# liaoherui/StrainScan

Hardware: AMD Instinct MI355X
Metric: M reads/sec vs 1433-strain E. coli DB (higher is better)
Workload: dtype u64

## Files before the change

### strainscan_amd/csrc/ss_common.h

```cpp
#pragma once
#include <hip/hip_runtime.h>
#include <stdint.h>
#include <stdio.h>
#include <atomic>
#include <functional>
#include <vector>
#include <string.h>

#include "strainscan_hip.h"

namespace ss {

void set_last_error(const char *what, const char *file, int line, hipError_t e);

#define SS_HIP(call)                                               \
    do {                                                           \
        hipError_t _e = (call);                                    \
        if (_e != hipSuccess) {                                    \
            ss::set_last_error(#call, __FILE__, __LINE__, _e);     \
            return (_e == hipErrorOutOfMemory) ? SS_ENOMEM         \
                   : (_e == hipErrorNoDevice)  ? SS_ENODEV         \
                                               : SS_EHIP;          \
        }                                                          \
    } while (0)
// ... 51 lines not shown
    uint32_t n_dir = 0;
    uint32_t n_dir_alloc = 0;
    uint32_t *d_bloom = nullptr;
    uint32_t bloom_bits = 0;
    uint64_t n_buckets = 0;
    uint32_t *d_counts = nullptr;
    int expect_hits = 0;
    uint64_t probe_set = 0;
    int probe_comb = 0;
    double probe_runs_per_tile = 0;
    uint32_t *d_slot_of_row = nullptr;
    uint8_t *d_row_valid = nullptr;
    char *h_stage[2] = {nullptr, nullptr};
    char *d_stage[2] = {nullptr, nullptr};
    uint64_t stage_bytes = 0;
    hipStream_t streams[2] = {nullptr, nullptr};
    hipEvent_t stage_free[2] = {nullptr, nullptr};
    std::atomic<uint64_t> launches{0};
    struct Worker { char *h_buf = nullptr; char *d_buf = nullptr; hipEvent_t done = nullptr; uint64_t cap = 0;
                    char *t_buf = nullptr; uint64_t t_cap = 0; };
    static constexpr int MAX_WORKERS = 64;
    Worker workers[MAX_WORKERS];
    static void free_workers(Worker *w, int n);
    uint64_t device_bytes = 0;
};

#include <chrono>
#include <mutex>

namespace ss { hipError_t big_malloc(void **p, uint64_t bytes, uint64_t *got = nullptr); void big_put(void *p, uint64_t cap); }
struct ss_reads {
    struct Slab {
        char *d = nullptr; uint64_t cap = 0, used = 0; bool binned = false;
        bool packed = false; uint64_t n_pos = 0; uint32_t L = 0, slot = 0;
        uint64_t positions() const { return packed ? n_pos : used; }
    };
    std::vector<Slab> slabs;
    std::mutex mu;
    uint64_t n_records = 0, n_bases = 0, device_bytes = 0, n_blocks = 0;
    bool has_cut_record = false;
    uint64_t first_slab = 0;
    uint64_t serial = next_serial();
    static uint64_t next_serial() { static std::atomic<uint64_t> c{0}; return ++c; }

    static uint64_t padded(uint64_t len) { return (len + 1 + 15) & ~15ull; }
    void adopt(char *d, uint64_t cap, uint64_t len)
    {
        std::lock_guard<std::mutex> g(mu);
        Slab sl;
        sl.d = d; sl.cap = cap; sl.used = padded(len);
        if (!slabs.empty() && slabs.back().used < slabs.back().cap) slabs.insert(slabs.end() - 1, sl);
        else slabs.push_back(sl);
        device_bytes += cap;
        n_blocks++;
    }
    char *reserve(uint64_t len)
    {
        const uint64_t need = padded(len);
        std::lock_guard<std::mutex> g(mu);
        if (slabs.empty() || slabs.back().used + need > slabs.back().cap) {
            Slab sl;
            sl.cap = std::max<uint64_t>(need, slabs.empty() ? std::max<uint64_t>(first_slab, 64ull << 20) : 512ull << 20);
            const auto t0 = std::chrono::steady_clock::now();
            if (ss::big_malloc((void **)&sl.d, sl.cap, &sl.cap) != hipSuccess) return nullptr;
            if (getenv("SS_INGEST_TRACE"))
                fprintf(stderr, "[ingest] slab of %.0f MB: %.4f s\n", sl.cap / 1e6,
                        std::chrono::duration<double>(std::chrono::steady_clock::now() - t0).count());
            slabs.push_back(sl);
        }
        Slab &sl = slabs.back();
        char *p = sl.d + sl.used;
        sl.used += need;
        device_bytes += need;
        n_blocks++;
        return p;
    }
};


namespace ss {
int reads_order_for_locality(ss_reads *R, bool force = false);
int order_flat_dev(const char *src, uint64_t n, ss_reads::Slab *out);
extern std::atomic<long long> g_hook_ascii_slabs;
void reorder_release();
void reorder_counters(uint64_t out[2]);
void reorder_timing(double out[3]);
int build_mini(ss_db *db, const uint64_t *keys, const uint8_t *flags, uint64_t n_rows, int upper_keys);
int build_mini_dev(ss_db *db, const uint64_t *keys, const uint8_t *flags, uint64_t n_rows, int upper_keys);
int mark_solid(ss_db *db);
using BlockSink = std::function<int(const char *h_buf, char *d_buf, uint64_t len, hipStream_t stream)>;
int parse_file_parallel(ss_db::Worker *workers, const char *path, int shard_rank, int shard_world,
                        uint64_t *n_records, uint64_t *n_bases, bool *handled, const BlockSink &sink, bool copy = true);
int parse_text_parallel(ss_db::Worker *workers, const char *text, uint64_t n, const char *path, int shard_rank,
                        int shard_world, uint64_t *n_records, uint64_t *n_bases, bool *handled, const BlockSink &sink,
                        bool copy = true);
struct InflatedText { char *p = nullptr; uint64_t n = 0; };
bool inflate_whole(const char *path, uint64_t budget, char **text, uint64_t *len, int mode, unsigned threads);
uint64_t inflate_budget_bytes();
hipStream_t ingest_stream(unsigned i);
void free_later(char *p);
std::vector<InflatedText> inflate_gz_inputs(const char *const *paths, int n_paths);
bool gz_on_gpu();
int gz_policy();
bool gpu_gunzip(const uint8_t *in, uint64_t in_n, char **text_dev, uint64_t *len, void **lease, int fd);
void gpu_gunzip_done(void *lease);
hipStream_t call_stream_get();
void call_stream_put(hipStream_t s);
struct GzPiece { uint64_t at, len, keep; std::vector<uint8_t> carry; };
bool gz_range_active();
extern std::atomic<long long> g_hook_entry, g_hook_decline, g_hook_skip_chain;
uint64_t gz_range_ticket();
void gz_range_pass(uint64_t ticket);
bool gpu_gunzip_range(const uint8_t *in, uint64_t in_n, char **text_dev, void **lease, int fd, std::vector<GzPiece> *pieces,
                      uint64_t ticket, bool decline = false);
int gz_fastq_pieces_dev(const char *path, uint64_t ticket, const std::function<int(char *, uint64_t, uint64_t, uint64_t)> &flat);
int gz_fastq_to_flat_dev(const char *path, int shard_rank, int shard_world, char **d_flat, uint64_t *flat_len, uint64_t *flat_cap,
                         uint64_t *n_records, char **text, uint64_t *text_len);
int gz_inputs_on_device(const char *const *paths, int n_paths, int shard_rank, int shard_world,
                        const std::function<int(int, char *, uint64_t, uint64_t, uint64_t)> &flat, std::vector<InflatedText> &texts,
                        std::vector<char> &done);
int scan_file_parallel(ss_db *db, const char *path, uint64_t *n_records, uint64_t *n_bases, bool *handled, int shard_rank = 0,
                       int shard_world = 1);
int scan_text_parallel(ss_db *db, const char *text, uint64_t n, uint64_t *n_records, uint64_t *n_bases, bool *handled,
                       int shard_rank = 0, int shard_world = 1);
int launch_scan_mini(ss_db *db, const void *bases_dev, uint64_t n, hipStream_t stream, unsigned blocks,
                     uint64_t n_tiles, bool binned = false, uint64_t set_id = 0, bool packed = false);
int launch_scan_mini_multi(ss_db *const *dbs, int n_dbs, const void *bases_dev, uint64_t n, hipStream_t stream, bool binned,
                           bool packed = false);
enum { MULTI_BLOOM = 0, MULTI_EXPECT = 1, MULTI_PLAIN = 2 };
int multi_kind(const ss_db *db);
void pool_keep_at_least(uint64_t bytes);
namespace l2s {
inline hipStream_t stream() { return hipStreamPerThread; }
hipError_t dmalloc(void **p, size_t n);
inline hipError_t dfree(void *p) { return p ? hipFreeAsync(p, stream()) : hipSuccess; }
inline hipError_t copy(void *d, const void *s_, size_t n, hipMemcpyKind k)
{
    const hipError_t e = hipMemcpyAsync(d, s_, n, k, stream());
    return e != hipSuccess ? e : hipStreamSynchronize(stream());
}
inline hipError_t set(void *d, int v, size_t n) { return hipMemsetAsync(d, v, n, stream()); }
inline hipError_t sync() { return hipStreamSynchronize(stream()); }
}
constexpr uint64_t BIG_KEEP_MIN = 256ull << 20;
void *big_take(uint64_t bytes, uint64_t *cap = nullptr);
void big_put(void *p, uint64_t cap);
void big_release();
hipError_t big_malloc(void **p, uint64_t bytes, uint64_t *got);
bool upload_file_to_device(int fd, uint64_t n, uint8_t *d_dst);
int scan_flat_dev(ss_db *db, const void *bases_dev, uint64_t n, void *stream, bool binned, uint64_t set_id = 0, bool packed = false);
}
```

### strainscan_amd/csrc/ss_ginflate.hip

```cpp
#include "ss_common.h"

#include <fcntl.h>
#include <sys/stat.h>
#include <unistd.h>
#include <zlib.h>

#include <algorithm>
#include <chrono>
#include <atomic>
#include <condition_variable>
#include <mutex>
#include <thread>
#include <vector>
#include <functional>
#include <future>

namespace {

constexpr uint32_t WSIZE = 32768;
constexpr uint16_t UNRES = 0x8000;
#ifndef SS_GZ_RING
#define SS_GZ_RING 2048
#endif
#ifndef SS_GZ_LITBITS
// ... 2338 lines not shown
    static const uint8_t hdr[10] = {0x1f, 0x8b, 8, 0, 0, 0, 0, 0, 0, 0xff};
    memcpy(img.get(), hdr, 10);
    {
        const unsigned T = (unsigned)std::max<uint64_t>(1, std::min<uint64_t>(8, comp_n >> 24));
        std::atomic<bool> ok(true);
        std::vector<std::thread> pool;
        for (unsigned w = 0; w < T; w++)
            pool.emplace_back([&, w] {
                uint64_t a = comp_n * w / T;
                const uint64_t e = comp_n * (w + 1) / T;
                while (a < e) {
                    const ssize_t r = pread(fd, img.get() + 10 + a, (size_t)std::min<uint64_t>(e - a, 1u << 30), (off_t)(off + a));
                    if (r <= 0) { ok = false; return; }
                    a += (uint64_t)r;
                }
            });
        for (auto &th : pool) th.join();
        close(fd);
        if (!ok) { delete L; return SS_EIO; }
    }
    uint8_t *t8 = img.get() + 10 + comp_n;
    for (int q = 0; q < 4; q++) { t8[q] = (uint8_t)(crc >> (8 * q)); t8[4 + q] = (uint8_t)(usize >> (8 * q)); }
    char *d = nullptr;
    uint64_t len = 0;
    if (!ss::gpu_gunzip(img.get(), in_n, &d, &len, &L->gz, -1)) { delete L; return SS_ERANGE; }
    if (len != usize) { ss::gpu_gunzip_done(L->gz); delete L; return SS_EIO; }
    *d_data = d; *n = len; *lease = L;
    return SS_OK;
}
extern "C" int ss_npz_member_done(void *lease)
{
    NpzLease *L = static_cast<NpzLease *>(lease);
    if (!L) return SS_OK;
    if (L->gz) ss::gpu_gunzip_done(L->gz);
    if (L->d_buf) hipFree(L->d_buf);
    delete L;
    return SS_OK;
}

extern "C" int ss_crc32_repeat(uint32_t prefix_crc, int byte, uint64_t n, uint32_t *out)
{
    if (!out || byte < 0 || byte > 255) return SS_EINVAL;
    const unsigned char b = (unsigned char)byte;
    uLong pw = crc32(crc32(0L, Z_NULL, 0), &b, 1);
    uLong acc = prefix_crc;
    uint64_t len = 1;
    for (uint64_t m = n; m; m >>= 1, len <<= 1) {
        if (m & 1) acc = crc32_combine(acc, pw, (z_off_t)len);
        if (m >> 1) pw = crc32_combine(pw, pw, (z_off_t)len);
    }
    *out = (uint32_t)acc;
    return SS_OK;
}

extern "C" int ss_gz_warm_up(int n_files)
{
    std::vector<PinSet *> got;
    for (int i = 0; i < std::min(n_files, 2); i++) {
        PinSet *p = pin_get();
        if (!p) break;
        got.push_back(p);
    }
    const bool ok = (int)got.size() == std::min(n_files, 2);
    for (PinSet *p : got) pin_put(p);
    return ok ? SS_OK : SS_ENOMEM;
}

extern "C" int ss_gz_set_range(int rank, int world, uint64_t slice_bytes, ss_gz_chain_fn chain, void *user)
{
    if (world < 1 || rank < 0 || rank >= world) return SS_EINVAL;
    std::lock_guard<std::mutex> one(ss::g_range_mu);
    ss::g_range.rank = rank; ss::g_range.world = world; ss::g_range.slice_bytes = slice_bytes; ss::g_range.fn = chain; ss::g_range.user = user;
    return SS_OK;
}

extern "C" int ss_test_hook(int which, long long value)
{
    switch (which) {
    case 1: ss::g_hook_entry = value; return SS_OK;
    case 2: ss::g_hook_decline = value; return SS_OK;
    case 3: ss::g_hook_skip_chain = value; return SS_OK;
    case 4: ss::g_hook_generic_k = value; return SS_OK;
    case 5: ss::g_hook_ascii_slabs = value; return SS_OK;
    default: return SS_EINVAL;
    }
}

extern "C" int ss_gz_range_counters(uint64_t *files, uint64_t *pieces)
{
    if (files) *files = ss::g_range_files.load();
    if (pieces) *pieces = ss::g_range_pieces.load();
    return SS_OK;
}
```

### strainscan_amd/csrc/ss_reorder.hip

```cpp
#include "ss_common.h"

#include <mutex>
#include "ss_scan_dev.h"

#include <algorithm>
#include <chrono>
#include <vector>

namespace {

#ifndef SS_ORDER_CH
#define SS_ORDER_CH 64
#endif
constexpr int CH = SS_ORDER_CH;
constexpr int RB = 256 * CH;
constexpr int HALO = 512;
static_assert(22 <= 23, "a table entry has 24 bits for the bin; order_bits stays at or below 22");
constexpr uint32_t NO_NL = 0xFFFFFFFFu;
constexpr int TCAP = 2 * CH;

__device__ __forceinline__ uint32_t nl_mask16(const uint4 v)
{
    const uint32_t w[4] = {v.x, v.y, v.z, v.w};
    uint32_t z[4];
#pragma unroll
    for (int d = 0; d < 4; d++) {
        const uint32_t x = w[d] ^ 0x0A0A0A0Au;
        z[d] = ~(((x & 0x7F7F7F7Fu) + 0x7F7F7F7Fu) | x) & 0x80808080u;
    }
    const uint32_t lo = __builtin_amdgcn_udot4(z[1], 0x80402010u, __builtin_amdgcn_udot4(z[0], 0x08040201u, 0u, false), false);
    const uint32_t hi = __builtin_amdgcn_udot4(z[3], 0x80402010u, __builtin_amdgcn_udot4(z[2], 0x08040201u, 0u, false), false);
    return (lo >> 7) | ((hi >> 7) << 8);
}

__device__ __forceinline__ uint4 load16_nl(const char *__restrict__ b, uint64_t i, uint64_t n)
{
    if (i + 16 <= n) { uint4 v; __builtin_memcpy(&v, b + i, 16); return v; }
    uint32_t w[4] = {0x0A0A0A0Au, 0x0A0A0A0Au, 0x0A0A0A0Au, 0x0A0A0A0Au};
    for (int k = 0; k < 16 && i + k < n; k++) {
        const uint32_t ch = (uint8_t)b[i + k];
        w[k >> 2] = (w[k >> 2] & ~(0xFFu << (8 * (k & 3)))) | (ch << (8 * (k & 3)));
    }
    return make_uint4(w[0], w[1], w[2], w[3]);
}

__device__ __forceinline__ uint32_t record_bin(const char *__restrict__ b, uint64_t s, uint64_t len, int bits)
{
    if (len < 31) return 1u << bits;
    uint4 q[2];
    __builtin_memcpy(q, b + s, 32);
    const uint32_t w[8] = {q[0].x, q[0].y, q[0].z, q[0].w, q[1].x, q[1].y, q[1].z, q[1].w};
    uint64_t km = 0;
    uint32_t bad = 0;
#pragma unroll
    for (int d = 0; d < 8; d++) {
        const uint32_t c = (w[d] >> 1) & 0x03030303u;
        const uint32_t letter = __builtin_amdgcn_perm(0u, 0x47544341u, c);
        uint32_t diff = (w[d] & 0xDFDFDFDFu) ^ letter;
        if (d == 7) diff &= 0x00FFFFFFu;
        bad |= diff;
        km |= (uint64_t)__builtin_amdgcn_udot4(c, 0x40100401u, 0u, false) << (8 * d);
    }
    if (bad) return 1u << bits;
    km &= 0x3FFFFFFFFFFFFFFFull;
    uint32_t best = 0xFFFFFFFFu;
#pragma unroll
    for (int i = 0; i < 31 - ss::MINI_M + 1; i++) {
        const uint32_t x = (uint32_t)(km >> (2 * i));
        best = min(best, (ss::mmkey(x) & ss::KEY_MASK) | (uint32_t)i);
    }
    const uint32_t x = (uint32_t)(km >> (2 * (best & 31u))) & ss::M30;
    return ss::mix30(x) >> (30 - bits);
}

__device__ __forceinline__ uint32_t wave_incl_sum(uint32_t v, int lane)
{
#pragma unroll
    for (int off = 1; off < 64; off <<= 1) {
        const uint32_t o = (uint32_t)__shfl_up((int)v, off, 64);
        if (lane >= off) v += o;
    }
    return v;
}

constexpr uint32_t T_OVERFLOW = 0xFFFFFFFFu;
constexpr int START_BITS = CH == 64 ? 14 : 15, LEN_BITS = 40 - START_BITS;
constexpr uint32_t LEN_LIMIT = 1u << LEN_BITS;
static_assert(RB == 1 << START_BITS, "a table entry holds the start within the tile in START_BITS bits");

struct TileLds {
    uint32_t first[5];
    uint32_t wcnt[4];
    uint32_t more;
    uint64_t src[256], dst[256];
    uint32_t len[256], bin[256], pend[256];
};

#if SS_ORDER_CH == 128
typedef unsigned __int128 mask_t;
__device__ __forceinline__ uint32_t mask_ctz(mask_t m) { const uint64_t lo = (uint64_t)m; return lo ? (uint32_t)__builtin_ctzll(lo) : 64u + (uint32_t)__builtin_ctzll((uint64_t)(m >> 64)); }
#else
typedef uint64_t mask_t;
__device__ __forceinline__ uint32_t mask_ctz(mask_t m) { return (uint32_t)__builtin_ctzll(m); }
#endif
struct TileState { mask_t nl, st; uint32_t later; uint64_t tile0, i0; };

__device__ __forceinline__ void tile_setup(const char *__restrict__ b, uint64_t n, TileLds &L, TileState &S)
{
    const int t = threadIdx.x, lane = t & 63, wave = t >> 6;
    S.tile0 = (uint64_t)blockIdx.x * RB;
    S.i0 = S.tile0 + (uint64_t)t * CH;
    mask_t nl = ~(mask_t)0;
    uint32_t prev = 1u;
    if (S.i0 < n) {
        uint4 v[CH / 16];
#pragma unroll
        for (int k = 0; k < CH / 16; k++) v[k] = load16_nl(b, S.i0 + 16u * k, n);
        prev = S.i0 == 0 ? 1u : (uint32_t)(b[S.i0 - 1] == '\n');
        nl = 0;
#pragma unroll
        for (int k = 0; k < CH / 16; k++) nl |= (mask_t)nl_mask16(v[k]) << (16 * k);
    }
    uint32_t suf = nl ? (uint32_t)t * CH + mask_ctz(nl) : NO_NL;
#pragma unroll
    for (int off = 1; off < 64; off <<= 1) {
        const uint32_t o = (uint32_t)__shfl_down((int)suf, off, 64);
// ... 339 lines not shown
            if (p < total) store_piece(dst, (((uint64_t)hi << 32) | lo) + off[r], v[r], L, slot, off[r]);
        }
    }
}

constexpr uint32_t PK_LDS = 4352;
constexpr int FPK = 4;

__global__ __launch_bounds__(256, 6) void place_fixed_packed_kernel(const char *__restrict__ b, uint64_t n, uint64_t n_rec, uint32_t L,
                                                                    uint32_t P, uint32_t magic_p, uint32_t A, uint32_t G, uint32_t ND,
                                                                    uint32_t magic_nd, unsigned long long *__restrict__ cursor,
                                                                    const uint32_t *__restrict__ bins, uint8_t *__restrict__ dst)
{
    __shared__ uint32_t lds[4][PK_LDS / 4 + 1];
    const int lane = threadIdx.x & 63, wave = threadIdx.x >> 6;
    const uint64_t r0 = ((uint64_t)blockIdx.x * 4u + (uint32_t)wave) * 64u;
    if (r0 >= n_rec) return;
    const uint32_t L1 = L + 1u, nr = (uint32_t)min((uint64_t)64, n_rec - r0), slot = slot_of(L), B = slot / 8u * 3u;
    const uint64_t base = r0 * L1;
    uint32_t *W = lds[wave];
    uint8_t *W8 = reinterpret_cast<uint8_t *>(W);
    unsigned long long d0 = 0;
    if ((uint32_t)lane < nr) d0 = atomicAdd(&cursor[bins[r0 + lane]], (unsigned long long)slot);
    for (uint32_t c0 = 0; c0 < nr; c0 += G) {
        const uint32_t nc = min(G, nr - c0), total = nc * P;
        for (uint32_t p0 = 0; p0 < total; p0 += 64u * FPK) {
            uint4 v[FPK];
#pragma unroll
            for (int r = 0; r < FPK; r++) {
                const uint32_t p = p0 + (uint32_t)lane + 64u * r, rec = min(__umulhi(p, magic_p), nc - 1u), off = (p - rec * P) * 16u;
                v[r] = make_uint4(0x0A0A0A0Au, 0x0A0A0A0Au, 0x0A0A0A0Au, 0x0A0A0A0Au);
                if (p < total && L > off) v[r] = load16_nl(b, base + (uint64_t)(c0 + rec) * L1 + off, n);
            }
#pragma unroll
            for (int r = 0; r < FPK; r++) {
                const uint32_t p = p0 + (uint32_t)lane + 64u * r, rec = min(__umulhi(p, magic_p), nc - 1u), off = (p - rec * P) * 16u;
                if (p >= total) continue;
                uint32_t w[4] = {v[r].x, v[r].y, v[r].z, v[r].w};
                const int keep = (int)min(16u, L > off ? L - off : 0u);
                if (keep < 16) {
#pragma unroll
                    for (int d = 0; d < 4; d++) {
                        const int k = keep - 4 * d;
                        if (k <= 0) w[d] = 0x0A0A0A0Au;
                        else if (k < 4) { const uint32_t m = (1u << (8 * k)) - 1u; w[d] = (w[d] & m) | (0x0A0A0A0Au & ~m); }
                    }
                }
                uint32_t code, inv;
                ss::dev::encode16(w, code, inv);
                uint16_t *q = reinterpret_cast<uint16_t *>(W8 + rec * A + 4u + (off >> 4) * 6u);
                q[0] = (uint16_t)code;
                q[1] = (uint16_t)((inv & 0xFFu) | ((code >> 8) & 0xFF00u));
                q[2] = (uint16_t)((code >> 24) | (inv & 0xFF00u));
            }
        }
        __builtin_amdgcn_fence(__ATOMIC_RELEASE, "wavefront");
        __builtin_amdgcn_wave_barrier();
        __builtin_amdgcn_fence(__ATOMIC_ACQUIRE, "wavefront");
        const uint32_t items = nc * ND;
        for (uint32_t i0 = 0; i0 < items; i0 += 64u) {
            const uint32_t i = i0 + (uint32_t)lane, rec = min(__umulhi(i, magic_nd), nc - 1u), jl = i - rec * ND;
            const uint32_t lo = (uint32_t)__shfl((int)(uint32_t)d0, (int)(c0 + rec), 64), hi = (uint32_t)__shfl((int)(uint32_t)(d0 >> 32), (int)(c0 + rec), 64);
            const uint64_t D = ((((uint64_t)hi << 32) | lo) >> 3) * 3u;
            const int o = (int)(4u * jl) - (int)(D & 3u);
            if (i < items && o < (int)B) {
                const uint32_t x = rec * A + 4u + (uint32_t)o;
                const uint32_t val = __builtin_amdgcn_alignbyte(W[(x >> 2) + 1u], W[x >> 2], x & 3u);
                uint8_t *out = dst + (D & ~3ull) + 4u * jl;
                if (o >= 0 && o + 4 <= (int)B) {
                    *reinterpret_cast<uint32_t *>(__builtin_assume_aligned(out, 4)) = val;
                } else {
#pragma unroll
                    for (int k = 0; k < 4; k++)
                        if (o + k >= 0 && o + k < (int)B) out[k] = (uint8_t)(val >> (8 * k));
                }
            }
        }
        __builtin_amdgcn_fence(__ATOMIC_RELEASE, "wavefront");
        __builtin_amdgcn_wave_barrier();
        __builtin_amdgcn_fence(__ATOMIC_ACQUIRE, "wavefront");
    }
}

constexpr int SCAN_PER = 4096;

__global__ __launch_bounds__(1024) void scan_sums_kernel(const unsigned long long *__restrict__ v, uint32_t n, unsigned long long *__restrict__ sums)
{
    __shared__ unsigned long long s_w[16];
    const int t = threadIdx.x, lane = t & 63, wave = t >> 6;
    const uint32_t i0 = blockIdx.x * SCAN_PER + (uint32_t)t * 4u;
    unsigned long long x = 0;
    for (uint32_t i = i0; i < min(n, i0 + 4u); i++) x += v[i];
#pragma unroll
    for (int off = 32; off > 0; off >>= 1) x += (unsigned long long)__shfl_xor((long long)x, off, 64);
    if (lane == 0) s_w[wave] = x;
    __syncthreads();
    if (t == 0) { unsigned long long r = 0; for (int w = 0; w < 16; w++) r += s_w[w]; sums[blockIdx.x] = r; }
}

__global__ __launch_bounds__(1024) void scan_top_kernel(unsigned long long *__restrict__ sums, uint32_t nb, unsigned long long *__restrict__ total)
{
    __shared__ unsigned long long s_part[1024];
    const int t = threadIdx.x;
    const uint32_t per = (nb + 1023u) / 1024u, a = min(nb, (uint32_t)t * per), e = min(nb, a + per);
    unsigned long long sum = 0;
    for (uint32_t i = a; i < e; i++) sum += sums[i];
    s_part[t] = sum;
    __syncthreads();
    if (t == 0) {
        unsigned long long run = 0;
        for (int i = 0; i < 1024; i++) { const unsigned long long v = s_part[i]; s_part[i] = run; run += v; }
        *total = run;
    }
    __syncthreads();
    unsigned long long run = s_part[t];
    for (uint32_t i = a; i < e; i++) { const unsigned long long v = sums[i]; sums[i] = run; run += v; }
}

__global__ __launch_bounds__(1024) void scan_apply_kernel(unsigned long long *__restrict__ v, uint32_t n, const unsigned long long *__restrict__ sums)
{
    __shared__ unsigned long long s_w[16];
    const int t = threadIdx.x, lane = t & 63, wave = t >> 6;
    const uint32_t i0 = blockIdx.x * SCAN_PER + (uint32_t)t * 4u;
    unsigned long long x[4], mine = 0;
#pragma unroll
    for (int k = 0; k < 4; k++) { x[k] = i0 + k < n ? v[i0 + k] : 0ull; mine += x[k]; }
    unsigned long long incl = mine;
#pragma unroll
    for (int off = 1; off < 64; off <<= 1) {
        const unsigned long long o = (unsigned long long)__shfl_up((long long)incl, off, 64);
        if (lane >= off) incl += o;
    }
    if (lane == 63) s_w[wave] = incl;
    __syncthreads();
    unsigned long long run = sums[blockIdx.x] + incl - mine;
    for (int w = 0; w < wave; w++) run += s_w[w];
#pragma unroll
    for (int k = 0; k < 4; k++) { if (i0 + k < n) v[i0 + k] = run; run += x[k]; }
}

int order_bits(uint64_t n_bytes)
{
    int bits = 12;
    while (bits < 22 && (n_bytes / 152) >> (bits + 2)) bits++;
    return bits;
}

}

namespace ss {

static std::mutex g_scr_mu;
static uint64_t g_order_n[2] = {0, 0};
static double g_order_ms[3] = {0, 0, 0};
static char *g_scr = nullptr;
static uint64_t g_scr_cap = 0;

std::atomic<long long> g_hook_ascii_slabs{0};

int order_flat_dev(const char *src, uint64_t n, ss_reads::Slab *out)
{
    *out = ss_reads::Slab();
    const int bits = order_bits(n);
    const uint32_t n_bins = (1u << bits) + 1u;
    static const bool trace = getenv("SS_INGEST_TRACE") != nullptr;
    const auto t_begin = std::chrono::steady_clock::now();
    auto lap = [&](const char *what) {
        if (!trace) return;
        hipDeviceSynchronize();
        fprintf(stderr, "[reorder] %-22s at %.4f s\n", what, std::chrono::duration<double>(std::chrono::steady_clock::now() - t_begin).count());
    };
    const unsigned nb = (unsigned)((n + RB - 1) / RB), nsb = (n_bins + SCAN_PER - 1) / SCAN_PER;
    const uint64_t o_sums = ((uint64_t)n_bins + 3) * 8, o_cnt = o_sums + (((uint64_t)nsb + 1) * 8), o_tab = (o_cnt + (uint64_t)nb * 4 + 255) & ~255ull;
    uint32_t fix_L = 0;
    uint64_t n_rec = 0;
    static const bool fixed_allowed = [] { const char *e = getenv("SS_ORDER_FIXED"); return !(e && !strcmp(e, "0")); }();
    if (fixed_allowed && n >= 64) {
        char head[FIX_MAX_L + 2];
        const size_t hn = (size_t)std::min<uint64_t>(n, sizeof(head));
        if (hipMemcpy(head, src, hn, hipMemcpyDeviceToHost) != hipSuccess) { ss::set_last_error("hipMemcpy", __FILE__, __LINE__, hipGetLastError()); return SS_EHIP; }
        const void *nl = memchr(head, '\n', hn);
        if (nl) {
            const uint32_t L = (uint32_t)((const char *)nl - head);
            if (L >= FIX_MIN_L && L <= FIX_MAX_L && n / (L + 1) >= 1 && n - (n / (L + 1)) * (L + 1) < 64) { fix_L = L; n_rec = n / (L + 1); }
        }
    }
    const uint64_t scratch = o_tab + std::max<uint64_t>((uint64_t)nb * TCAP * 8, (n_rec * 4 + 255) & ~255ull);
    char *d_scr = nullptr, *d_new = nullptr;
#define SS_R(call) do { if ((call) != hipSuccess) { ss::set_last_error(#call, __FILE__, __LINE__, hipGetLastError()); hipFree(d_scr); hipFree(d_new); return SS_EHIP; } } while (0)
    uint64_t scr_cap = 0;
    {
        std::lock_guard<std::mutex> g(g_scr_mu);
        if (g_scr && g_scr_cap >= scratch) { d_scr = g_scr; scr_cap = g_scr_cap; g_scr = nullptr; g_scr_cap = 0; }
    }
    if (!d_scr) { SS_R(hipMalloc((void **)&d_scr, scratch)); scr_cap = scratch; }
    unsigned long long *d_hist = (unsigned long long *)d_scr, *d_sums = (unsigned long long *)(d_scr + o_sums);
    uint32_t *d_cnt = (uint32_t *)(d_scr + o_cnt);
    unsigned long long *d_tab = (unsigned long long *)(d_scr + o_tab);
    constexpr unsigned pad1 = 0, pad2 = 0;
    unsigned long long tail[3] = {0, 0, 0};
    bool fixed = false, packed = false;
    if (fix_L) {
        const uint32_t L1 = fix_L + 1u, P = (::slot_of(fix_L) + 15u) >> 4;
        const unsigned nbf = (unsigned)((n_rec + 255) / 256);
        SS_R(hipMemsetAsync(d_hist, 0, o_sums, 0));
        hipLaunchKernelGGL(count_fixed_kernel, dim3(nbf), dim3(256), 0, 0, src, n, n_rec, fix_L, (uint32_t)(((1ull << 32) + L1 - 1) / L1), bits, d_hist,
                           (uint32_t *)d_tab, d_hist + n_bins + 1, d_hist + n_bins + 2);
        hipLaunchKernelGGL(scan_sums_kernel, dim3(nsb), dim3(1024), 0, 0, d_hist, n_bins, d_sums);
        hipLaunchKernelGGL(scan_top_kernel, dim3(1), dim3(1024), 0, 0, d_sums, nsb, d_hist + n_bins);
        hipLaunchKernelGGL(scan_apply_kernel, dim3(nsb), dim3(1024), 0, 0, d_hist, n_bins, d_sums);
        SS_R(hipMemcpy(tail, d_hist + n_bins, 24, hipMemcpyDeviceToHost));
        fixed = tail[1] == 0;
        packed = fixed && tail[2] == 0 && g_hook_ascii_slabs.load() == 0;
        (void)P;
    }
    if (!fixed) {
        SS_R(hipMemsetAsync(d_hist, 0, o_sums, 0));
        hipLaunchKernelGGL(count_kernel, dim3(nb), dim3(256), pad1, 0, src, n, bits, d_hist, d_cnt, d_tab, d_hist + n_bins + 1);
        hipLaunchKernelGGL(scan_sums_kernel, dim3(nsb), dim3(1024), 0, 0, d_hist, n_bins, d_sums);
        hipLaunchKernelGGL(scan_top_kernel, dim3(1), dim3(1024), 0, 0, d_sums, nsb, d_hist + n_bins);
        hipLaunchKernelGGL(scan_apply_kernel, dim3(nsb), dim3(1024), 0, 0, d_hist, n_bins, d_sums);
        SS_R(hipMemcpy(tail, d_hist + n_bins, 16, hipMemcpyDeviceToHost));
    }
    const unsigned long long total = tail[0];
    lap("count + prefix");
    const auto t_counted = std::chrono::steady_clock::now();
    const uint64_t cap = std::max<uint64_t>((total + 15) & ~15ull, 16);
    const uint64_t bytes = packed ? std::max<uint64_t>(ss::dev::in_bytes(true, cap) + 8, cap >= ss::BIG_KEEP_MIN ? cap : 0) : cap;
    uint64_t real_cap = bytes;
    SS_R(ss::big_malloc((void **)&d_new, bytes, &real_cap));
    const auto t_alloc = std::chrono::steady_clock::now();
    lap("new slab");
    if (packed) {
        const uint32_t P = (::slot_of(fix_L) + 15u) >> 4, B = ::slot_of(fix_L) / 8u * 3u, A = (6u * P + 8u + 3u) & ~3u;
        const uint32_t G = std::min<uint32_t>(64u, PK_LDS / A), ND = ((B + 2u) >> 2) + 1u;
        hipLaunchKernelGGL(place_fixed_packed_kernel, dim3((unsigned)((n_rec + 255) / 256)), dim3(256), 0, 0, src, n, n_rec, fix_L, P,
                           (uint32_t)(((1ull << 32) + P - 1) / P), A, G, ND, (uint32_t)(((1ull << 32) + ND - 1) / ND), d_hist,
                           (const uint32_t *)d_tab, (uint8_t *)d_new);
        const uint64_t t0 = total / 8u * 3u, t1 = ss::dev::in_bytes(true, cap) + 8;
        SS_R(hipMemsetAsync(d_new + t0, 0xFF, t1 - t0, 0));
        if (cap > total) SS_R(hipMemsetAsync(d_new + t0, 0x55, 2, 0));
    } else if (fixed) {
        const uint32_t P = (::slot_of(fix_L) + 15u) >> 4;
        hipLaunchKernelGGL(place_fixed_kernel, dim3((unsigned)((n_rec + 255) / 256)), dim3(256), 0, 0, src, n, n_rec, fix_L, (uint32_t)(((1ull << 32) + P - 1) / P),
                           d_hist, (const uint32_t *)d_tab, d_new);
    } else {
        hipLaunchKernelGGL(place_kernel, dim3(nb), dim3(256), pad2, 0, src, n, d_hist, d_cnt, d_tab, d_new);
        if (tail[1]) hipLaunchKernelGGL(place_again_kernel, dim3(nb), dim3(256), 0, 0, src, n, bits, d_hist, d_cnt, d_new);
    }
    if (!packed && cap > total) SS_R(hipMemsetAsync(d_new + total, '\n', cap - total, 0));
    SS_R(hipGetLastError());
    SS_R(hipDeviceSynchronize());
    lap("place");
    {
        const auto t_end = std::chrono::steady_clock::now();
        auto ms = [](std::chrono::steady_clock::time_point a, std::chrono::steady_clock::time_point b) { return std::chrono::duration<double, std::milli>(b - a).count(); };
        std::lock_guard<std::mutex> g(g_scr_mu);
        g_order_ms[0] = ms(t_begin, t_counted); g_order_ms[1] = ms(t_counted, t_alloc); g_order_ms[2] = ms(t_alloc, t_end);
        g_order_n[fixed ? 0 : 1]++;
    }
#undef SS_R
    {
        std::lock_guard<std::mutex> g(g_scr_mu);
        if (!g_scr || g_scr_cap < scr_cap) { std::swap(g_scr, d_scr); std::swap(g_scr_cap, scr_cap); }
    }
    if (d_scr) hipFree(d_scr);
    out->d = d_new; out->cap = real_cap; out->binned = true;
    out->used = packed ? ss::dev::in_bytes(true, cap) : cap;
    if (packed) { out->packed = true; out->n_pos = cap; out->L = fix_L; out->slot = ::slot_of(fix_L); }
    return SS_OK;
}

void reorder_timing(double out[3])
{
    std::lock_guard<std::mutex> g(g_scr_mu);
    for (int i = 0; i < 3; i++) out[i] = g_order_ms[i];
}

void reorder_counters(uint64_t out[2])
{
    std::lock_guard<std::mutex> g(g_scr_mu);
    out[0] = g_order_n[0]; out[1] = g_order_n[1];
}

void reorder_release()
{
    char *d = nullptr;
    {
        std::lock_guard<std::mutex> g(g_scr_mu);
        std::swap(d, g_scr);
        g_scr_cap = 0;
    }
    if (d) hipFree(d);
}

bool reads_order_wanted()
{
    const char *e = getenv("SS_READS_ORDER");
    return !(e && (!strcmp(e, "file") || !strcmp(e, "0") || !strcmp(e, "off")));
}

int reads_order_for_locality(ss_reads *R, bool force)
{
    if (!R) return SS_EINVAL;
    if (!force && !reads_order_wanted()) return SS_OK;
    uint64_t bytes = 0;
    size_t mem_free = 0, mem_total = 0;
    const bool known = hipMemGetInfo(&mem_free, &mem_total) == hipSuccess;
    for (auto &sl : R->slabs) {
        const bool room = known && mem_free > sl.used + sl.used / 8 + (1ull << 30);
        if (sl.used >= 64 && (room || force)) {
            ss_reads::Slab nsl;
            const int rc = order_flat_dev(sl.d, sl.used, &nsl);
            if (rc) return rc;
            ss::big_put(sl.d, sl.cap);
            sl = nsl;
        }
        bytes += sl.cap;
    }
    R->device_bytes = bytes;
    return SS_OK;
}

}
```

Before: 2887.

## Bin fixed-length reads via key radix sort and permuted gather instead of atomic histogram

Result: faster. 3076, median of 6 (+6.6%).

```diff
diff --git a/strainscan_amd/csrc/ss_common.h b/strainscan_amd/csrc/ss_common.h
--- a/strainscan_amd/csrc/ss_common.h
+++ b/strainscan_amd/csrc/ss_common.h
@@ -157,6 +157,7 @@
 int reads_order_for_locality(ss_reads *R, bool force = false);
 int order_flat_dev(const char *src, uint64_t n, ss_reads::Slab *out);
 extern std::atomic<long long> g_hook_ascii_slabs;
+extern std::atomic<long long> g_hook_atomic_binning;
 void reorder_release();
 void reorder_counters(uint64_t out[2]);
 void reorder_timing(double out[3]);
diff --git a/strainscan_amd/csrc/ss_ginflate.hip b/strainscan_amd/csrc/ss_ginflate.hip
--- a/strainscan_amd/csrc/ss_ginflate.hip
+++ b/strainscan_amd/csrc/ss_ginflate.hip
@@ -2444,6 +2444,7 @@
     case 3: ss::g_hook_skip_chain = value; return SS_OK;
     case 4: ss::g_hook_generic_k = value; return SS_OK;
     case 5: ss::g_hook_ascii_slabs = value; return SS_OK;
+    case 6: ss::g_hook_atomic_binning = value; return SS_OK;
     default: return SS_EINVAL;
     }
 }
diff --git a/strainscan_amd/csrc/ss_reorder.hip b/strainscan_amd/csrc/ss_reorder.hip
--- a/strainscan_amd/csrc/ss_reorder.hip
+++ b/strainscan_amd/csrc/ss_reorder.hip
@@ -2,6 +2,8 @@
 
 #include <mutex>
 #include "ss_scan_dev.h"
+
+#include <hipcub/hipcub.hpp>
 
 #include <algorithm>
 #include <chrono>
@@ -42,6 +44,17 @@
         w[k >> 2] = (w[k >> 2] & ~(0xFFu << (8 * (k & 3)))) | (ch << (8 * (k & 3)));
     }
     return make_uint4(w[0], w[1], w[2], w[3]);
+}
+
+__device__ __forceinline__ uint4 load16_clamped(const char *__restrict__ b, uint64_t i, uint64_t n)
+{
+    uint4 v;
+    if (i + 16 <= n) { __builtin_memcpy(&v, b + i, 16); return v; }
+    unsigned __int128 x;
+    __builtin_memcpy(&x, b + n - 16, 16);
+    x >>= 8u * (uint32_t)(i + 16 - n);
+    __builtin_memcpy(&v, &x, 16);
+    return v;
 }
 
 __device__ __forceinline__ uint32_t record_bin(const char *__restrict__ b, uint64_t s, uint64_t len, int bits)
@@ -547,6 +560,111 @@
     }
 }
 
+__global__ __launch_bounds__(256) void key_fixed_kernel(const char *__restrict__ b, uint64_t n, uint64_t n_rec, uint32_t L, int bits,
+                                                        uint32_t *__restrict__ key, uint32_t *__restrict__ val,
+                                                        unsigned long long *__restrict__ not_fixed)
+{
+    const uint64_t i = (uint64_t)blockIdx.x * 256u + threadIdx.x;
+    if (i >= n_rec) return;
+    const uint64_t s = i * (L + 1u);
+    bool bad = i > 0 && b[s - 1] != '\n';
+    if (i + 1 == n_rec)
+        for (uint64_t k = s + L; k < n; k++) bad |= b[k] != '\n';
+    key[i] = record_bin(b, s, L, bits);
+    val[i] = (uint32_t)i;
+    const uint64_t m = __ballot(bad);
+    if (m && (uint32_t)(threadIdx.x & 63) == (uint32_t)__builtin_ctzll(m) &&
+        !*(volatile unsigned long long *)not_fixed) atomicOr(not_fixed, 1ull);
+}
+
+constexpr uint32_t GX_LDS_PK = 6144, GX_LDS_ASCII = 8192;
+constexpr int GPK = 3;
+
+inline uint32_t gather_rows(bool pk, uint32_t L)
+{
+    const uint32_t slot = slot_of(L), R = pk ? slot / 8u * 3u : slot, lim = pk ? GX_LDS_PK : GX_LDS_ASCII;
+    uint32_t G = 64;
+    while (G > 1 && (G * R > lim || (G * R) % 16u)) G--;
+    return G;
+}
+
+template <bool PK>
+__global__ __launch_bounds__(256, 7) void gather_fixed_kernel(const char *__restrict__ b, uint64_t n, uint64_t n_rec, uint32_t L,
+                                                              uint32_t P, uint32_t magic_p, uint32_t G, const uint32_t *__restrict__ perm,
+                                                              uint8_t *__restrict__ dst, unsigned long long *__restrict__ not_fixed,
+                                                              unsigned long long *__restrict__ not_packable)
+{
+    extern __shared__ uint4 gx_lds[];
+    const int lane = threadIdx.x & 63, wave = threadIdx.x >> 6;
+    const uint64_t r0 = ((uint64_t)blockIdx.x * 4u + (uint32_t)wave) * 64u;
+    if (r0 >= n_rec || *(volatile unsigned long long *)not_fixed || (PK && *(volatile unsigned long long *)not_packable)) return;
+    const uint32_t L1 = L + 1u, nr = (uint32_t)min((uint64_t)64, n_rec - r0), slot = slot_of(L), R = PK ? slot / 8u * 3u : slot;
+    uint4 *W = gx_lds + (size_t)wave * (G * R / 16u);
+    uint8_t *W8 = reinterpret_cast<uint8_t *>(W);
+    const uint32_t mine = (uint32_t)lane < nr ? perm[r0 + lane] : 0u;
+    bool bad = false;
+    uint32_t alpha = 0;
+    for (uint32_t c0 = 0; c0 < nr; c0 += G) {
+        const uint32_t nc = min(G, nr - c0), total = nc * P;
+        for (uint32_t p0 = 0; p0 < total; p0 += 64u * GPK) {
+            uint4 v[GPK];
+#pragma unroll
+            for (int r = 0; r < GPK; r++) {
+                const uint32_t p = p0 + (uint32_t)lane + 64u * r, rec = min(__umulhi(p, magic_p), nc - 1u), off = (p - rec * P) * 16u;
+                const uint32_t s = (uint32_t)__shfl((int)mine, (int)(c0 + rec), 64);
+                v[r] = make_uint4(0x0A0A0A0Au, 0x0A0A0A0Au, 0x0A0A0A0Au, 0x0A0A0A0Au);
+                if (p < total && L >= off) v[r] = load16_clamped(b, (uint64_t)s * L1 + off, n);
+            }
+#pragma unroll
+            for (int r = 0; r < GPK; r++) {
+                const uint32_t p = p0 + (uint32_t)lane + 64u * r, rec = min(__umulhi(p, magic_p), nc - 1u), off = (p - rec * P) * 16u;
+                if (p >= total) continue;
+                uint32_t w[4] = {v[r].x, v[r].y, v[r].z, v[r].w};
+                if (L >= off) {
+                    const uint32_t m = nl_mask16(v[r]), e = L - off;
+                    const uint32_t want = e < 16u ? 1u << e : 0u, valid = e < 16u ? (2u << e) - 1u : 0xFFFFu;
+                    bad |= ((m ^ want) & valid) != 0u;
+                }
+                const int keep = (int)min(16u, L > off ? L - off : 0u);
+                if (keep < 16) {
+#pragma unroll
+                    for (int d = 0; d < 4; d++) {
+                        const int k = keep - 4 * d;
+                        if (k <= 0) w[d] = 0x0A0A0A0Au;
+                        else if (k < 4) { const uint32_t mk = (1u << (8 * k)) - 1u; w[d] = (w[d] & mk) | (0x0A0A0A0Au & ~mk); }
+                    }
+                }
+                if (PK) {
+                    alpha |= not_packable4(w[0]) | not_packable4(w[1]) | not_packable4(w[2]) | not_packable4(w[3]);
+                    uint32_t code, inv;
+                    ss::dev::encode16(w, code, inv);
+                    uint8_t *q = W8 + rec * R + (off >> 4) * 6u;
+                    q[0] = (uint8_t)code; q[1] = (uint8_t)(code >> 8); q[2] = (uint8_t)inv;
+                    if (off + 16u <= slot) { q[3] = (uint8_t)(code >> 16); q[4] = (uint8_t)(code >> 24); q[5] = (uint8_t)(inv >> 8); }
+                } else {
+                    uint64_t *q = reinterpret_cast<uint64_t *>(W8 + rec * R + off);
+                    q[0] = (uint64_t)w[0] | ((uint64_t)w[1] << 32);
+                    if (off + 16u <= slot) q[1] = (uint64_t)w[2] | ((uint64_t)w[3] << 32);
+                }
+            }
+        }
+        __builtin_amdgcn_fence(__ATOMIC_RELEASE, "wavefront");
+        __builtin_amdgcn_wave_barrier();
+        __builtin_amdgcn_fence(__ATOMIC_ACQUIRE, "wavefront");
+        const uint32_t span = nc * R;
+        uint8_t *out = dst + (r0 + c0) * R;
+        for (uint32_t q = (uint32_t)lane * 16u; q < span; q += 1024u) {
+            if (q + 16u <= span) *reinterpret_cast<uint4 *>(__builtin_assume_aligned(out + q, 16)) = W[q >> 4];
+            else for (uint32_t k = q; k < span; k++) out[k] = W8[k];
+        }
+        __builtin_amdgcn_fence(__ATOMIC_RELEASE, "wavefront");
+        __builtin_amdgcn_wave_barrier();
+        __builtin_amdgcn_fence(__ATOMIC_ACQUIRE, "wavefront");
+    }
+    if (__ballot(bad) && lane == 0 && !*(volatile unsigned long long *)not_fixed) atomicOr(not_fixed, 1ull);
+    if (PK && __ballot(alpha != 0u) && lane == 0 && !*(volatile unsigned long long *)not_packable) atomicOr(not_packable, 1ull);
+}
+
 constexpr int SCAN_PER = 4096;
 
 __global__ __launch_bounds__(1024) void scan_sums_kernel(const unsigned long long *__restrict__ v, uint32_t n, unsigned long long *__restrict__ sums)
@@ -622,6 +740,7 @@
 static uint64_t g_scr_cap = 0;
 
 std::atomic<long long> g_hook_ascii_slabs{0};
+std::atomic<long long> g_hook_atomic_binning{0};
 
 int order_flat_dev(const char *src, uint64_t n, ss_reads::Slab *out)
 {
@@ -650,7 +769,16 @@
             if (L >= FIX_MIN_L && L <= FIX_MAX_L && n / (L + 1) >= 1 && n - (n / (L + 1)) * (L + 1) < 64) { fix_L = L; n_rec = n / (L + 1); }
         }
     }
-    const uint64_t scratch = o_tab + std::max<uint64_t>((uint64_t)nb * TCAP * 8, (n_rec * 4 + 255) & ~255ull);
+    const bool sorted = fix_L && g_hook_atomic_binning.load() == 0 && n_rec < (1ull << 31);
+    const uint64_t a4 = (n_rec * 4 + 255) & ~255ull;
+    size_t sort_tb = 0;
+    if (sorted) {
+        hipcub::DoubleBuffer<uint32_t> k(nullptr, nullptr), v(nullptr, nullptr);
+        if (hipcub::DeviceRadixSort::SortPairs(nullptr, sort_tb, k, v, (int)n_rec, 0, bits + 1) != hipSuccess) {
+            ss::set_last_error("hipcub::DeviceRadixSort::SortPairs", __FILE__, __LINE__, hipGetLastError()); return SS_EHIP;
+        }
+    }
+    const uint64_t scratch = o_tab + std::max<uint64_t>((uint64_t)nb * TCAP * 8, sorted ? 4 * a4 + ((sort_tb + 255) & ~255ull) : a4);
     char *d_scr = nullptr, *d_new = nullptr;
 #define SS_R(call) do { if ((call) != hipSuccess) { ss::set_last_error(#call, __FILE__, __LINE__, hipGetLastError()); hipFree(d_scr); hipFree(d_new); return SS_EHIP; } } while (0)
     uint64_t scr_cap = 0;
@@ -665,8 +793,72 @@
     constexpr unsigned pad1 = 0, pad2 = 0;
     unsigned long long tail[3] = {0, 0, 0};
     bool fixed = false, packed = false;
-    if (fix_L) {
-        const uint32_t L1 = fix_L + 1u, P = (::slot_of(fix_L) + 15u) >> 4;
+    uint64_t cap = 0, real_cap = 0;
+    auto t_counted = t_begin, t_alloc = t_begin;
+    float ms_key_sort = -1.f;
+    auto block_bytes = [](bool pk, uint64_t c) { return pk ? std::max<uint64_t>(ss::dev::in_bytes(true, c) + 8, c >= ss::BIG_KEEP_MIN ? c : 0) : c; };
+    auto fill_tail = [&](bool pk, uint64_t total) -> hipError_t {
+        hipError_t e = hipSuccess;
+        if (pk) {
+            const uint64_t t0 = total / 8u * 3u, t1 = ss::dev::in_bytes(true, cap) + 8;
+            e = hipMemsetAsync(d_new + t0, 0xFF, t1 - t0, 0);
+            if (e == hipSuccess && cap > total) e = hipMemsetAsync(d_new + t0, 0x55, 2, 0);
+        } else if (cap > total) {
+            e = hipMemsetAsync(d_new + total, '\n', cap - total, 0);
+        }
+        return e;
+    };
+    if (sorted) {
+        const uint32_t slot = ::slot_of(fix_L), P = (slot + 15u) >> 4;
+        const uint64_t total = n_rec * slot;
+        cap = std::max<uint64_t>((total + 15) & ~15ull, 16);
+        const bool want_packed = g_hook_ascii_slabs.load() == 0;
+        SS_R(ss::big_malloc((void **)&d_new, block_bytes(want_packed, cap), &real_cap));
+        t_alloc = std::chrono::steady_clock::now();
+        lap("new slab");
+        uint32_t *k0 = (uint32_t *)(d_scr + o_tab), *k1 = (uint32_t *)(d_scr + o_tab + a4), *v0 = (uint32_t *)(d_scr + o_tab + 2 * a4),
+                 *v1 = (uint32_t *)(d_scr + o_tab + 3 * a4);
+        void *d_temp = d_scr + o_tab + 4 * a4;
+        unsigned long long *flags = d_hist + n_bins;
+        hipEvent_t ev[2] = {nullptr, nullptr};
+        SS_R(hipEventCreate(&ev[0]));
+        if (hipEventCreate(&ev[1]) != hipSuccess) { hipEventDestroy(ev[0]); SS_R(hipErrorOutOfMemory); }
+        auto gather = [&](bool pk, const uint32_t *perm) {
+            const uint32_t G = gather_rows(pk, fix_L), R = pk ? slot / 8u * 3u : slot;
+            auto kern = pk ? gather_fixed_kernel<true> : gather_fixed_kernel<false>;
+            hipLaunchKernelGGL(kern, dim3((unsigned)((n_rec + 255) / 256)), dim3(256), 4u * G * R, 0, src, n, n_rec, fix_L, P,
+                               (uint32_t)(((1ull << 32) + P - 1) / P), G, perm, (uint8_t *)d_new, flags + 1, flags + 2);
+        };
+        hipError_t e = hipMemsetAsync(flags, 0, 24, 0);
+        if (e == hipSuccess) e = hipEventRecord(ev[0], 0);
+        if (e == hipSuccess) {
+            hipLaunchKernelGGL(key_fixed_kernel, dim3((unsigned)((n_rec + 255) / 256)), dim3(256), 0, 0, src, n, n_rec, fix_L, bits, k0, v0, flags + 1);
+            hipcub::DoubleBuffer<uint32_t> dk(k0, k1), dv(v0, v1);
+            e = hipcub::DeviceRadixSort::SortPairs(d_temp, sort_tb, dk, dv, (int)n_rec, 0, bits + 1, 0);
+            if (e == hipSuccess) e = hipEventRecord(ev[1], 0);
+            const uint32_t *perm = dv.Current();
+            if (e == hipSuccess) { gather(want_packed, perm); e = fill_tail(want_packed, total); }
+            if (e == hipSuccess) e = hipMemcpy(tail + 1, flags + 1, 16, hipMemcpyDeviceToHost);
+            fixed = tail[1] == 0;
+            if (e == hipSuccess && fixed && want_packed && tail[2]) {
+                if (real_cap < cap) {
+                    ss::big_put(d_new, real_cap); d_new = nullptr;
+                    e = ss::big_malloc((void **)&d_new, cap, &real_cap);
+                }
+                if (e == hipSuccess) { gather(false, perm); e = fill_tail(false, total); }
+                if (e == hipSuccess) e = hipMemcpy(tail + 1, flags + 1, 8, hipMemcpyDeviceToHost);
+                fixed = tail[1] == 0;
+            }
+        }
+        if (e == hipSuccess) e = hipGetLastError();
+        if (e == hipSuccess && fixed) e = hipEventElapsedTime(&ms_key_sort, ev[0], ev[1]);
+        hipEventDestroy(ev[0]); hipEventDestroy(ev[1]);
+        SS_R(e);
+        packed = fixed && want_packed && tail[2] == 0;
+        tail[0] = total;
+        if (!fixed) { ss::big_put(d_new, real_cap); d_new = nullptr; }
+    } else if (fix_L) {
+        const uint32_t L1 = fix_L + 1u;
         const unsigned nbf = (unsigned)((n_rec + 255) / 256);
         SS_R(hipMemsetAsync(d_hist, 0, o_sums, 0));
         hipLaunchKernelGGL(count_fixed_kernel, dim3(nbf), dim3(256), 0, 0, src, n, n_rec, fix_L, (uint32_t)(((1ull << 32) + L1 - 1) / L1), bits, d_hist,
@@ -677,7 +869,6 @@
         SS_R(hipMemcpy(tail, d_hist + n_bins, 24, hipMemcpyDeviceToHost));
         fixed = tail[1] == 0;
         packed = fixed && tail[2] == 0 && g_hook_ascii_slabs.load() == 0;
-        (void)P;
     }
     if (!fixed) {
         SS_R(hipMemsetAsync(d_hist, 0, o_sums, 0));
@@ -688,32 +879,29 @@
         SS_R(hipMemcpy(tail, d_hist + n_bins, 16, hipMemcpyDeviceToHost));
     }
     const unsigned long long total = tail[0];
-    lap("count + prefix");
-    const auto t_counted = std::chrono::steady_clock::now();
-    const uint64_t cap = std::max<uint64_t>((total + 15) & ~15ull, 16);
-    const uint64_t bytes = packed ? std::max<uint64_t>(ss::dev::in_bytes(true, cap) + 8, cap >= ss::BIG_KEEP_MIN ? cap : 0) : cap;
-    uint64_t real_cap = bytes;
-    SS_R(ss::big_malloc((void **)&d_new, bytes, &real_cap));
-    const auto t_alloc = std::chrono::steady_clock::now();
-    lap("new slab");
-    if (packed) {
-        const uint32_t P = (::slot_of(fix_L) + 15u) >> 4, B = ::slot_of(fix_L) / 8u * 3u, A = (6u * P + 8u + 3u) & ~3u;
-        const uint32_t G = std::min<uint32_t>(64u, PK_LDS / A), ND = ((B + 2u) >> 2) + 1u;
-        hipLaunchKernelGGL(place_fixed_packed_kernel, dim3((unsigned)((n_rec + 255) / 256)), dim3(256), 0, 0, src, n, n_rec, fix_L, P,
-                           (uint32_t)(((1ull << 32) + P - 1) / P), A, G, ND, (uint32_t)(((1ull << 32) + ND - 1) / ND), d_hist,
-                           (const uint32_t *)d_tab, (uint8_t *)d_new);
-        const uint64_t t0 = total / 8u * 3u, t1 = ss::dev::in_bytes(true, cap) + 8;
-        SS_R(hipMemsetAsync(d_new + t0, 0xFF, t1 - t0, 0));
-        if (cap > total) SS_R(hipMemsetAsync(d_new + t0, 0x55, 2, 0));
-    } else if (fixed) {
-        const uint32_t P = (::slot_of(fix_L) + 15u) >> 4;
-        hipLaunchKernelGGL(place_fixed_kernel, dim3((unsigned)((n_rec + 255) / 256)), dim3(256), 0, 0, src, n, n_rec, fix_L, (uint32_t)(((1ull << 32) + P - 1) / P),
-                           d_hist, (const uint32_t *)d_tab, d_new);
-    } else {
-        hipLaunchKernelGGL(place_kernel, dim3(nb), dim3(256), pad2, 0, src, n, d_hist, d_cnt, d_tab, d_new);
-        if (tail[1]) hipLaunchKernelGGL(place_again_kernel, dim3(nb), dim3(256), 0, 0, src, n, bits, d_hist, d_cnt, d_new);
-    }
-    if (!packed && cap > total) SS_R(hipMemsetAsync(d_new + total, '\n', cap - total, 0));
+    if (!(sorted && fixed)) {
+        lap("count + prefix");
+        t_counted = std::chrono::steady_clock::now();
+        cap = std::max<uint64_t>((total + 15) & ~15ull, 16);
+        SS_R(ss::big_malloc((void **)&d_new, block_bytes(packed, cap), &real_cap));
+        t_alloc = std::chrono::steady_clock::now();
+        lap("new slab");
+        if (packed) {
+            const uint32_t P = (::slot_of(fix_L) + 15u) >> 4, B = ::slot_of(fix_L) / 8u * 3u, A = (6u * P + 8u + 3u) & ~3u;
+            const uint32_t G = std::min<uint32_t>(64u, PK_LDS / A), ND = ((B + 2u) >> 2) + 1u;
+            hipLaunchKernelGGL(place_fixed_packed_kernel, dim3((unsigned)((n_rec + 255) / 256)), dim3(256), 0, 0, src, n, n_rec, fix_L, P,
+                               (uint32_t)(((1ull << 32) + P - 1) / P), A, G, ND, (uint32_t)(((1ull << 32) + ND - 1) / ND), d_hist,
+                               (const uint32_t *)d_tab, (uint8_t *)d_new);
+        } else if (fixed) {
+            const uint32_t P = (::slot_of(fix_L) + 15u) >> 4;
+            hipLaunchKernelGGL(place_fixed_kernel, dim3((unsigned)((n_rec + 255) / 256)), dim3(256), 0, 0, src, n, n_rec, fix_L, (uint32_t)(((1ull << 32) + P - 1) / P),
+                               d_hist, (const uint32_t *)d_tab, d_new);
+        } else {
+            hipLaunchKernelGGL(place_kernel, dim3(nb), dim3(256), pad2, 0, src, n, d_hist, d_cnt, d_tab, d_new);
+            if (tail[1]) hipLaunchKernelGGL(place_again_kernel, dim3(nb), dim3(256), 0, 0, src, n, bits, d_hist, d_cnt, d_new);
+        }
+        SS_R(fill_tail(packed, total));
+    }
     SS_R(hipGetLastError());
     SS_R(hipDeviceSynchronize());
     lap("place");
@@ -721,7 +909,11 @@
         const auto t_end = std::chrono::steady_clock::now();
         auto ms = [](std::chrono::steady_clock::time_point a, std::chrono::steady_clock::time_point b) { return std::chrono::duration<double, std::milli>(b - a).count(); };
         std::lock_guard<std::mutex> g(g_scr_mu);
-        g_order_ms[0] = ms(t_begin, t_counted); g_order_ms[1] = ms(t_counted, t_alloc); g_order_ms[2] = ms(t_alloc, t_end);
+        if (sorted && fixed) {
+            g_order_ms[0] = ms_key_sort; g_order_ms[1] = ms(t_begin, t_alloc); g_order_ms[2] = ms(t_alloc, t_end) - ms_key_sort;
+        } else {
+            g_order_ms[0] = ms(t_begin, t_counted); g_order_ms[1] = ms(t_counted, t_alloc); g_order_ms[2] = ms(t_alloc, t_end);
+        }
         g_order_n[fixed ? 0 : 1]++;
     }
 #undef SS_R
```
